# zellerlab/GECCO

Hardware: AMD Instinct MI355X
Metric: genes/sec CRF decode (windowed fwd-bwd marginals + Viterbi) (higher is better)
Workload: dtype f64

## Files before the change

gecco_amd/_native.py:

```python
import ctypes
import operator
import os
from typing import Optional, Sequence

import numpy as np

_HERE = os.path.dirname(os.path.abspath(__file__))
LIB_PATH = os.path.join(_HERE, "lib", "libgecco_crf.so")

OK, EINVAL, EFORMAT, ENOMEM, EHIP, ENODEV, EUNSUPPORTED = 0, -1, -2, -3, -4, -5, -6

_c_i32p = ctypes.POINTER(ctypes.c_int32)
_c_f64p = ctypes.POINTER(ctypes.c_double)
_c_u8p = ctypes.POINTER(ctypes.c_uint8)
_c_i8p = ctypes.POINTER(ctypes.c_int8)
_c_u32p = ctypes.POINTER(ctypes.c_uint32)
_vp = ctypes.c_void_p

SIGNATURES = {
    "gecco_crf_last_error": (ctypes.c_char_p, []),
    "gecco_crf_version": (ctypes.c_int, []),
    "gecco_crf_model_load": (ctypes.c_int, [ctypes.c_char_p, ctypes.c_size_t, ctypes.POINTER(_vp)]),
    "gecco_crf_model_from_tables": (ctypes.c_int, [_c_f64p, _c_f64p, ctypes.c_int32, ctypes.c_int32, ctypes.POINTER(_vp)]),
    "gecco_crf_model_free": (None, [_vp]),
# ... 103 lines not shown
         _c_f64p, _c_f64p, _c_f64p, _c_f64p, _c_f64p, _c_f64p],
    ),
    "gecco_crf_segment": (
        ctypes.c_int,
        [ctypes.c_int32, _c_f64p, _c_u8p, _c_i32p, ctypes.c_int32, ctypes.c_double, ctypes.c_int32, ctypes.c_int32,
         ctypes.c_int32, ctypes.c_int32, _c_i32p, ctypes.c_int32, _c_i32p],
    ),
    "gecco_crf_segment_ex": (
        ctypes.c_int, [ctypes.c_int32, _c_f64p, _c_u8p, _c_i32p, ctypes.c_int32, _vp, _c_i32p, ctypes.c_int32, _c_i32p]
    ),
    "gecco_crf_domain_composition": (
        ctypes.c_int,
        [ctypes.c_int32, _c_i32p, ctypes.c_int32, _c_i32p, ctypes.c_int32, _c_i32p, _c_f64p, ctypes.c_int32, ctypes.c_int32, _c_f64p],
    ),
    "gecco_crf_plan_create": (
        ctypes.c_int, [_vp, ctypes.c_int32, _c_i32p, ctypes.c_int32, ctypes.c_int32, ctypes.c_int32, ctypes.c_int32, ctypes.POINTER(_vp)]
    ),
    "gecco_crf_plan_free": (None, [_vp]),
    "gecco_crf_plan_num_genes": (ctypes.c_int32, [_vp]),
    "gecco_crf_plan_num_windows": (ctypes.c_int64, [_vp]),
    "gecco_crf_plan_num_tiles": (ctypes.c_int32, [_vp]),
    "gecco_crf_plan_tile_out": (ctypes.c_int32, [_vp]),
    "gecco_crf_plan_kernel_name": (ctypes.c_char_p, [_vp]),
    "gecco_crf_plan_run_windowed": (ctypes.c_int, [_vp, _vp, _vp, ctypes.c_int32, _vp, _vp]),
    "gecco_crf_plan_run_windowed_all": (ctypes.c_int, [_vp, _vp, _vp, ctypes.c_int32, _vp, _vp, _vp]),
    "gecco_crf_plan_all_kernel_name": (ctypes.c_char_p, [_vp]),
    "gecco_crf_plan_time_windowed_all": (
        ctypes.c_int, [_vp, _vp, _vp, ctypes.c_int32, _vp, _vp, _vp, ctypes.c_int32, ctypes.c_int32, ctypes.POINTER(ctypes.c_float)]
    ),
    "gecco_crf_plan_run_decode": (ctypes.c_int, [_vp, _vp, _vp, ctypes.c_int32, _vp, _vp, _vp, _vp]),
    "gecco_crf_plan_run_decode_pipelined": (ctypes.c_int, [_vp, _vp, _vp, ctypes.c_int32, _vp, _vp, _vp, _vp]),
    "gecco_crf_plan_run_marginals_full": (ctypes.c_int, [_vp, _vp, _vp, _vp, _vp, _vp]),
    "gecco_crf_plan_run_viterbi": (ctypes.c_int, [_vp, _vp, _vp, _vp, _vp, _vp]),
    "gecco_crf_plan_run_segment": (
        ctypes.c_int,
        [_vp, _vp, _vp, ctypes.c_double, ctypes.c_int32, ctypes.c_int32, ctypes.c_int32, ctypes.c_int32, _vp, ctypes.c_int32, _vp, _vp],
    ),
    "gecco_crf_plan_run_segment_ex": (ctypes.c_int, [_vp, _vp, _vp, _vp, _vp, ctypes.c_int32, _vp, _vp]),
    "gecco_crf_host_alloc": (ctypes.c_int, [ctypes.c_size_t, ctypes.POINTER(_vp)]),
    "gecco_crf_host_free": (None, [_vp]),
    "gecco_crf_session_create": (ctypes.c_int, [_vp, _c_i32p, ctypes.c_int32, ctypes.POINTER(_vp)]),
    "gecco_crf_session_free": (None, [_vp]),
    "gecco_crf_session_set_chunk_genes": (ctypes.c_int, [_vp, ctypes.c_int32]),
    "gecco_crf_session_set_direct_genes": (ctypes.c_int, [_vp, ctypes.c_int32]),
    "gecco_crf_session_stats": (
        ctypes.c_int,
# ... 1247 lines not shown
        if h:
            self._lib.gecco_crf_plan_free(h)

    @property
    def num_genes(self) -> int:
        return self._lib.gecco_crf_plan_num_genes(self._h)

    @property
    def num_windows(self) -> int:
        return self._lib.gecco_crf_plan_num_windows(self._h)

    @property
    def num_tiles(self) -> int:
        return self._lib.gecco_crf_plan_num_tiles(self._h)

    @property
    def tile_out(self) -> int:
        return self._lib.gecco_crf_plan_tile_out(self._h)

    @property
    def kernel_name(self) -> str:
        return self._lib.gecco_crf_plan_kernel_name(self._h).decode()

    def run_windowed(self, d_gene_ptr: int, d_attr_id: int, d_p_out: int, label=1, stream: int = 0):
        _check(self._lib.gecco_crf_plan_run_windowed(self._h, d_gene_ptr, d_attr_id, int(label), d_p_out, stream or None))

    @property
    def all_kernel_name(self) -> str:
        return self._lib.gecco_crf_plan_all_kernel_name(self._h).decode()

    def run_windowed_all(self, d_gene_ptr: int, d_attr_id: int, d_p_all: int, d_p_any: int = 0, background=None, stream: int = 0):
        _check(self._lib.gecco_crf_plan_run_windowed_all(self._h, d_gene_ptr, d_attr_id, -1 if background is None else int(background),
                                                         d_p_all, d_p_any or None, stream or None))

    def time_windowed_all(self, d_gene_ptr: int, d_attr_id: int, d_p_all: int, d_p_any: int = 0, background=None, stream: int = 0,
                          warmup=2, iters=10) -> float:
        ms = ctypes.c_float(0)
        _check(self._lib.gecco_crf_plan_time_windowed_all(self._h, d_gene_ptr, d_attr_id, -1 if background is None else int(background),
                                                          d_p_all, d_p_any or None, stream or None, int(warmup), int(iters),
                                                          ctypes.byref(ms)))
        return ms.value

    def run_decode(self, d_gene_ptr: int, d_attr_id: int, d_p_out: int, d_y: int, label: int = 1, d_score: int = 0, stream: int = 0):
        _check(self._lib.gecco_crf_plan_run_decode(self._h, d_gene_ptr, d_attr_id or None, int(label), d_p_out, d_y,
                                                   d_score or None, stream or None))

# ... 440 lines not shown
```

gecco_amd/csrc/capi.cpp:

```cpp
#include <cmath>
#include <cstdlib>
#include <cstring>
#include <exception>
#include <limits>
#include <memory>
#include <new>
#include <string>
#include <vector>

#include "../../include/gecco_crf.h"
#include "crf_exact_exp.hpp"
#include "crf_fisher.hpp"
#include "crf_forest.hpp"
#include "crf_model.hpp"
#include "crf_overlap.hpp"
#include "crf_plan.hpp"
#include "crf_session.hpp"
#include "crf_tables.hpp"
#include "crf_train.hpp"

using namespace gecco;

struct gecco_crf_model {
    Model m;
// ... 161 lines not shown
    }
    if (n_contigs > 0 && contig_ptr && contig_ptr[0] != 0) {
        set_error("contig_ptr[0] must be 0");
        return GECCO_CRF_EINVAL;
    }
    DeviceScope guard;
    GECCO_GUARD_BEGIN
    std::unique_ptr<gecco_crf_plan> h(new gecco_crf_plan());
    int rc = plan_build(m->m, device, contig_ptr, n_contigs, window, step, pad, h->p);
    if (rc) return rc;
    *out = h.release();
    return GECCO_CRF_OK;
    GECCO_GUARD_END
}
GECCO_API void gecco_crf_plan_free(gecco_crf_plan *p) {
    DeviceScope guard;
    delete p;
}
GECCO_API int32_t gecco_crf_plan_num_genes(const gecco_crf_plan *p) { return p ? p->p.n_genes : 0; }
GECCO_API int64_t gecco_crf_plan_num_windows(const gecco_crf_plan *p) { return p ? p->p.n_windows : 0; }
GECCO_API int32_t gecco_crf_plan_num_tiles(const gecco_crf_plan *p) { return p ? p->p.ntiles : 0; }
GECCO_API int32_t gecco_crf_plan_tile_out(const gecco_crf_plan *p) { return p ? p->p.tile_out : 0; }
GECCO_API const char *gecco_crf_plan_kernel_name(const gecco_crf_plan *p) { return p ? p->p.kernel_name.c_str() : ""; }

GECCO_API int gecco_crf_plan_run_windowed(gecco_crf_plan *p, const int32_t *d_gene_ptr, const int32_t *d_attr_id,
                                          int32_t label, double *d_p_out, void *stream) {
    if (!p) return GECCO_CRF_EINVAL;
    DeviceScope guard;
    GECCO_GUARD_BEGIN
    return plan_run_windowed(p->p, {d_gene_ptr, d_attr_id}, label, d_p_out, static_cast<hipStream_t>(stream));
    GECCO_GUARD_END
}

GECCO_API int gecco_crf_plan_run_windowed_all(gecco_crf_plan *p, const int32_t *d_gene_ptr, const int32_t *d_attr_id,
                                              int32_t background, double *d_p_all, double *d_p_any, void *stream) {
    if (!p) return GECCO_CRF_EINVAL;
    DeviceScope guard;
    GECCO_GUARD_BEGIN
    return plan_run_windowed_all(p->p, {d_gene_ptr, d_attr_id}, background, d_p_all, d_p_any, static_cast<hipStream_t>(stream));
    GECCO_GUARD_END
}
GECCO_API const char *gecco_crf_plan_all_kernel_name(const gecco_crf_plan *p) { return p ? plan_all_kernel_name(p->p) : ""; }

template <class Call>
static int time_calls(hipStream_t s, int32_t warmup, int32_t iters, float *ms_per_launch, Call call) {
    int rc;
// ... 2016 lines not shown
```

gecco_amd/csrc/crf_device.hpp:

```cpp
#pragma once
#include <hip/hip_runtime.h>

#include <cstddef>
#include <cstdint>

namespace gecco {

struct WinArgs {
    const int32_t *gene_ptr;
    const int32_t *attr_id;
    const double2 *wtab2;
    const double *wtab;
    const int32_t *c_slot;
    const int32_t *c_gene;
    const int32_t *c_n;
    const int4 *tile_desc;
    const uint64_t *start_bits;
    double *p_out;
    double2 *state_out;
    double *dstate_out;
    int32_t K, S, ntiles, W, step, L, label;
    int32_t n_genes, A;
    int32_t tiles_per_wg;
    int32_t all_regular;
    uint32_t rescale_mask;
    double mu01, rho, kappa_over_mu01, inv_kappa;
    double expc[12];
    double ratio_zmax;
    double g00, g01, g10, g11;
    int32_t generic;
    const double *exp_trans;
    double *scratch;
    const double *rtab;
    const double2 *ptab;
    int32_t prod_cnt;
    int32_t csr_end, csr_begin;
};

constexpr int kWinThreads = 256;
constexpr int kWinMaxW = 32;
constexpr int kWinTilesPerWg = 2;
constexpr int kWinTiles1MaxSlots = 350000;

__device__ __forceinline__ double exp_neg(double t, const double (&kExpC)[12]) {
    const double n = rint(t * 1.4426950408889634);
    double r = fma(n, 0.6931471805599453094, -t);
    r = fma(n, 2.3190468138462996e-17, r);
    double p = kExpC[0];
#pragma unroll
    for (int i = 1; i < 12; ++i) p = fma(p, r, kExpC[i]);
    p = fma(p, r, 1.0);
    p = fma(p, r, 1.0);
    return ldexp(p, -int(n));
}

__device__ __forceinline__ double exp_signed(double x, const double (&kExpC)[12]) {
    const double n = rint(x * 1.4426950408889634);
    double r = fma(-n, 0.6931471805599453094, x);
    r = fma(-n, 2.3190468138462996e-17, r);
// ... 311 lines not shown
```

gecco_amd/csrc/crf_kernels.hip:

```cpp
#include "crf_device.hpp"
#include "crf_lanes.hpp"
#include "crf_vd_short.hpp"

namespace gecco {
namespace {

typedef double f64x2 __attribute__((ext_vector_type(2)));

__device__ __forceinline__ double max_nocanon(double a, double b) {
    double r;
    asm("v_max_f64 %0, %1, %2" : "=v"(r) : "v"(a), "v"(b));
    return r;
}

__device__ __forceinline__ int xcd_remap(int orig, int nwg) {
    const int xcd = orig & 7, q = nwg >> 3, r = nwg & 7;
    const int base = xcd < r ? xcd * (q + 1) : r * (q + 1) + (xcd - r) * q;
    return base + (orig >> 3);
}

__device__ __forceinline__ void store_wt(double *p, double v) {
    __hip_atomic_store(reinterpret_cast<unsigned long long *>(p), static_cast<unsigned long long>(__double_as_longlong(v)),
                       __ATOMIC_RELAXED, __HIP_MEMORY_SCOPE_AGENT);
}

__device__ __forceinline__ double lds_read1(const double *p) {
    return __longlong_as_double(static_cast<long long>(
        __hip_atomic_load(reinterpret_cast<const unsigned long long *>(p), __ATOMIC_RELAXED, __HIP_MEMORY_SCOPE_WORKGROUP)));
}

__device__ __forceinline__ void rescale_pair(double &u, double &v) {
    int ex;
    (void)frexp(fmax(u, v), &ex);
    u = ldexp(u, -ex);
    v = ldexp(v, -ex);
}


constexpr int kGatherUnroll = 8;

template <int WMAX, int NT, int TT, bool EXACT>
struct WinSmem {
    static constexpr int JMAX = TT == 1 ? 2 : TT;
    static constexpr int CAP = TT == 1 ? NT + WMAX - 1 : TT * NT;
    static constexpr int CMAX = EXACT ? CAP / WMAX + 3 : CAP + 2;
    f64x2 ef[2 * CAP];
    uint32_t ginfo[CAP];
    f64x2 carry[NT / 64][WMAX];
    int32_t cslot[CMAX];
    int32_t cgene[CMAX];
    int32_t cn[CMAX];
};

struct SlotInfo {
    int gene;
    bool start_ok;
};

template <class Smem>
__device__ __forceinline__ SlotInfo slot_lookup(const Smem &sm, int cnt, int q, int S, int W, int step) {
    SlotInfo r{-1, false};
    if (q < 0 || q >= S) return r;
// ... 64 lines not shown
    using Smem = WinSmem<WMAX, NT, TT, EXACT>;
    constexpr int JMAX = Smem::JMAX;
    constexpr bool RATIO = !RESCALE && EXACT;
    const int W = EXACT ? WMAX : P.W;
    const int tid = threadIdx.x, lane = tid & 63, wave = tid >> 6;
    const int OUT = NT - (W - 1);
    const int ns = TT * OUT + 2 * (W - 1);
    const int q0 = tile * (TT * OUT) - (W - 1);

    const int4 td = P.all_regular ? make_int4(0, 0, 0, 1) : P.tile_desc[tile];
    int gene[JMAX];
    bool start[JMAX];
#pragma unroll
    for (int j = 0; j < JMAX; ++j) {
        gene[j] = -1;
        start[j] = false;
    }
    if (td.w & 1) {
#pragma unroll
        for (int j = 0; j < JMAX; ++j) {
            const int sl = tid + j * NT, q = q0 + sl;
            if (sl < ns && q >= 0 && q < P.S) {
                gene[j] = q + td.x;
                start[j] = (reinterpret_cast<const uint32_t *>(P.start_bits)[q >> 5] >> (q & 31)) & 1u;
            }
        }
    } else {
        const int cnt = td.z - td.y + 1;
        for (int j = tid; j <= cnt; j += NT) {
            sm.cslot[j] = P.c_slot[td.y + j];
            if (j < cnt) {
                sm.cgene[j] = P.c_gene[td.y + j];
                sm.cn[j] = P.c_n[td.y + j];
            }
        }
        __syncthreads();
#pragma unroll
        for (int j = 0; j < JMAX; ++j) {
            const int sl = tid + j * NT;
            if (sl < ns) {
                const SlotInfo si = slot_lookup(sm, cnt, q0 + sl, P.S, W, P.step);
                gene[j] = si.gene;
                start[j] = si.start_ok;
            }
        }
    }

// ... 30 lines not shown
        constexpr int SBASE = (Smem::CAP + 1) / 2;
        constexpr int APL = (2 * Smem::CAP - SBASE) / NT;
        constexpr int SCAP = APL * NT;
        static_assert(APL >= 1, "parking area smaller than one round of the workgroup");
        f64x2 *park = sm.ef + SBASE;
#pragma unroll 1
        for (uint32_t base = 0; base < n_attr; base += SCAP) {
            int id[APL];
#pragma unroll
            for (int a = 0; a < APL; ++a) id[a] = __builtin_amdgcn_raw_buffer_load_b32(ra, int((base + a * NT + tid) << 2), 0, 0);
            i32x4 w[APL];
#pragma unroll
            for (int a = 0; a < APL; ++a) {
                const uint32_t wo = min(uint32_t(id[a]), imax) << 4;
                w[a] = __builtin_amdgcn_raw_buffer_load_b128(rw, int(wo), 0, 0);
            }
#pragma unroll
            for (int a = 0; a < APL; ++a)
                park[a * NT + tid] = f64x2{__hiloint2double(w[a].y, w[a].x), __hiloint2double(w[a].w, w[a].z)};
            __syncthreads();
            const uint32_t c0 = lo_tile + base, c1 = c0 + SCAP;
#pragma unroll
            for (int j = 0; j < JMAX; ++j) {
                const f64x2 *k = park + (max(lo[j], c0) - c0);
                const f64x2 *const e = park + (min(hi[j], c1) - c0);
                for (; k < e && hi[j] > c0; ++k) {
                    const f64x2 v = *k;
                    if (RATIO) {
                        sc1[j] += v.x;
                        sc0[j] *= v.y;
                    } else {
                        sc0[j] += v.x;
                        sc1[j] += v.y;
                    }
                }
            }
            if (base + SCAP < n_attr) __syncthreads();
        }
        if (RATIO) {
#pragma unroll
            for (int j = 0; j < JMAX; ++j) long_run |= hi[j] - lo[j] > uint32_t(P.prod_cnt) ? 1u << j : 0u;
        }
        if (!RATIO && n_attr > 0) __syncthreads();
    } else {
        uint32_t off[JMAX], cnt[JMAX];
#pragma unroll
        for (int j = 0; j < JMAX; ++j) {
            int lo = 0, hi = 0;
            if (gene[j] >= 0) {
                lo = P.gene_ptr[gene[j]];
                hi = P.gene_ptr[gene[j] + 1];
            }
            off[j] = uint32_t(lo) - lo_tile;
            cnt[j] = uint32_t(hi - lo);
        }
        int ids[JMAX][kGatherUnroll];
#pragma unroll
// ... 31 lines not shown
            }
        }
    }
    if (RATIO) {
        if (__builtin_amdgcn_ballot_w64(long_run != 0) != 0) {
#pragma unroll
            for (int j = 0; j < JMAX; ++j)
                if ((long_run >> j) & 1u) sc0[j] = mu_exp_tab(sc1[j], P.rtab, P.expc);
        }
    }
    double *rr = reinterpret_cast<double *>(sm.ef);
#pragma unroll
    for (int j = 0; j < JMAX; ++j) {
        if (TT > 1 || j == 0 || wave == 0) {
            const int sl = tid + j * NT;
            const double s0 = sc0[j], s1 = sc1[j];
            if (sl >= W - 1 && sl < TT * OUT + (W - 1) && gene[j] >= 0) {
                if (!RATIO && P.state_out) reinterpret_cast<f64x2 *>(P.state_out)[gene[j]] = P.label ? f64x2{s0, s1} : f64x2{s1, s0};
            }
            const double d = RATIO ? s1 : s1 - s0;
            if (sl < ns) {
                if (RATIO) {
                    const double r = s0;
                    rr[sl] = __hiloint2double(__double2hiint(r) | (start[j] ? int(0x80000000u) : 0), __double2loint(r));
                    if (!(td.w & 1)) sm.ginfo[sl] = uint32_t(gene[j] + 1);
                } else {
                    const double e = exp_neg(fabs(d), P.expc);
                    const double e1 = d > 0.0 ? 1.0 : e;
                    sm.ef[sl] = f64x2{d > 0.0 ? e : 1.0, P.mu01 * e1};
                    sm.ginfo[sl] = (start[j] ? 0x80000000u : 0u) | uint32_t(gene[j] + 1);
                }
            }
        }
    }
    if (P.dstate_out) {
#pragma unroll
        for (int j = 0; j < JMAX; ++j) {
            if (TT > 1 || j == 0 || wave == 0) {
                const int sl = tid + j * NT;
                if (sl >= W - 1 && sl < TT * OUT + (W - 1) && gene[j] >= 0) {
                    const double d = RATIO ? sc1[j] : sc1[j] - sc0[j];
                    const double dd = __hiloint2double(__double2hiint(d) ^ (P.label ? 0 : int(0x80000000u)), __double2loint(d));
                    store_wt(P.dstate_out + gene[j], dd);
                }
            }
        }
    }
    __syncthreads();

    const uint32_t rmask = P.rescale_mask;
    const double rho = P.rho;
#pragma unroll 1
    for (int ph = 0; ph < TT; ++ph) {
        if (SMALL && ph > 0 && q0 + (W - 1) + ph * OUT >= P.S) break;
        const int sbase = ph * OUT + tid;
        bool my_start = false;
        int my_gene;
        if (RATIO) {
            const int q = q0 + sbase;
            my_gene = (td.w & 1) ? ((q >= 0 && q < P.S) ? q + td.x : -1) : int(sm.ginfo[sbase]) - 1;
        } else {
            const uint32_t gi = sm.ginfo[sbase];
            my_start = gi >> 31;
            my_gene = int(gi & 0x7fffffffu) - 1;
        }
        const f64x2 *ef = sm.ef + sbase;
        if constexpr (RATIO) {
            const double *rrs = rr + sbase;
            double A1[WMAX];
            const double r0 = lds_read1(rrs);
            double a0 = 1.0, a1 = fabs(r0) * P.kappa_over_mu01;
            A1[0] = a1;
#pragma unroll
            for (int k = 1; k < WMAX; ++k) {
                if (EXACT || k < W) {
                    const double r = fabs(lds_read1(rrs + k));
                    const double t = a0 + a1;
                    a1 = fma(a1, rho, a0) * r;
                    a0 = t;
                    A1[k] = a1;
                }
            }
            asm volatile("" ::: "memory");
            double z = fma(a1, P.inv_kappa, a0);
            const bool renorm = __builtin_amdgcn_ballot_w64(!(z < P.ratio_zmax)) != 0;
            auto pair_of = [&](double r, double &e0, double &f) {
                const bool pos = r > P.mu01;
                const double rc = fmin(r, 1.0e300);
                double q = __builtin_amdgcn_rcp(rc);
                q = fma(fma(-rc, q, 1.0), q, q);
// ... 2 lines not shown
            };
            if (renorm) {
                double e0, f;
                pair_of(fabs(r0), e0, f);
                a0 = e0;
                a1 = f * P.kappa_over_mu01;
                A1[0] = a1;
#pragma unroll
                for (int k = 1; k < WMAX; ++k) {
                    if (EXACT || k < W) {
                        pair_of(fabs(rrs[k]), e0, f);
                        const double t = a0 + a1;
                        a1 = fma(a1, rho, a0) * f;
                        a0 = t * e0;
                        A1[k] = a1;
                    }
                }
                z = fma(a1, P.inv_kappa, a0);
            }
            double b0, b1;
            {
                double r = __builtin_amdgcn_rcp(z);
                r = fma(fma(-z, r, 1.0), r, r);
                b0 = __double2hiint(r0) < 0 ? r : 0.0;
                b1 = b0 * P.inv_kappa;
            }
            double R = 0.0;
            double *carry = reinterpret_cast<double *>(&sm.carry[0][0]);
            if (!renorm) {
                double rcur = W > 1 ? lds_read1(rrs + (W - 1)) : 0.0;
#pragma unroll
                for (int k = WMAX - 1; k >= 0; --k) {
                    if (EXACT || k < W) {
                        double rnext = 0.0;
                        if (k > 1) rnext = lds_read1(rrs + (k - 1));
                        const double cand = A1[k] * b1;
                        if (k < W - 1) {
                            if (lane == 63 && wave < NT / 64 - 1) carry[wave * WMAX + k] = R;
                            R = wave_shr1_zero(R);
                        }
                        R = max_nocanon(R, cand);
                        if (k > 0) {
                            const double u = fabs(rcur) * b1;
                            b1 = fma(u, rho, b0);
                            b0 = b0 + u;
                        }
                        rcur = rnext;
                    }
                }
            } else {
#pragma unroll
                for (int k = WMAX - 1; k >= 0; --k) {
                    if (EXACT || k < W) {
                        const double cand = A1[k] * b1;
                        if (k < W - 1) {
                            if (lane == 63 && wave < NT / 64 - 1) carry[wave * WMAX + k] = R;
                            R = wave_shr1_zero(R);
                        }
                        R = max_nocanon(R, cand);
                        if (k > 0) {
                            double e0, f;
                            pair_of(fabs(rrs[k]), e0, f);
                            const double cc = e0 * b0, u = f * b1;
                            b0 = cc + u;
                            b1 = fma(u, rho, cc);
                        }
                    }
                }
            }
            __syncthreads();
            if (wave > 0 && lane < W - 1) {
                int t2 = tid;
                if (LEAN) asm volatile("" : "+v"(t2));
                R = fmax(R, carry[((t2 >> 6) - 1) * WMAX + (t2 & 63)]);
            }
            R = fmin(R, 1.0);
            if (tid >= W - 1 && my_gene >= 0) store_wt(P.p_out + my_gene, R);
        } else if constexpr (!RESCALE) {
            double A1[WMAX];
            double a0, a1;
            {
                const f64x2 c = ef[0];
                a0 = c.x;
                a1 = fabs(c.y) * P.kappa_over_mu01;
            }
            A1[0] = a1;
#pragma unroll
            for (int k = 1; k < WMAX; ++k) {
                if (EXACT || k < W) {
                    const f64x2 c = ef[k];
                    const double t = a0 + a1;
                    a1 = fma(a1, rho, a0) * fabs(c.y);
                    a0 = t * c.x;
                    A1[k] = a1;
                }
            }
            asm volatile("" ::: "memory");

            double b0, b1;
            {
// ... 84 lines not shown
            }
            if (tid >= W - 1 && my_gene >= 0) P.p_out[my_gene] = (Rx + Ry > 0.0) ? Rx / (Rx + Ry) : 0.0;
        }
        if (TT > 1) __syncthreads();
    }
}

template <int WMAX, bool EXACT, bool RESCALE, int NT, int TT>
__global__ void __launch_bounds__(NT, (RESCALE ? (WMAX <= 20 ? 5 : 3) : (WMAX <= 20 ? (TT <= 2 ? 8 : 5) : 3))) crf_windowed_l2(const WinArgs P) {
    __shared__ WinSmem<WMAX, NT, TT, EXACT> sm;
    windowed_tile<WMAX, EXACT, RESCALE, NT, TT>(P, sm, xcd_remap(blockIdx.x, P.ntiles));
}

__global__ void __launch_bounds__(kWinThreads, 4) crf_windowed_small_l2(const WinArgs P) {
    __shared__ WinSmem<20, kWinThreads, 2, true> sm;
    windowed_tile<20, true, false, kWinThreads, 2, false, true>(P, sm, 0);
}

struct PipeArgs {
    const int32_t *gene_ptr, *attr_id;
    const double2 *ptab;
    const int32_t *c_slot, *c_gene, *c_n;
    const int4 *tile_desc;
    const uint64_t *start_bits;
    double *p_out, *dstate_out;
    const double *rtab;
    int32_t S, ntiles, step, label, n_genes, A, all_regular, nvd8, prod_cnt;
    double mu01, rho, kappa_over_mu01, inv_kappa, ratio_zmax, expc5[5];
    const double *dstate;
    const uint8_t *flags;
    const uint16_t *lane_bits;
    const int32_t *cblk, *csr_gene_ptr, *csr_attr_id;
    const double2 *csr_wtab01;
    double2 *alpha;
    uint32_t *vd_stats;
    int8_t *y;
    int32_t s_n_genes, csr_n_attrs, v_exact, n_cblocks;
    double t00, t01, t10, t11, v_lo, v_hi, v_k, v_wmax2, v_tmax;
};

template <int TILES, int WGS>
__global__ void __launch_bounds__(kWinThreads, WGS) crf_decode_pipelined(const PipeArgs K) {
    using Smem = WinSmem<20, kWinThreads, TILES, true>;
    constexpr size_t kBytes = sizeof(Smem) > sizeof(VdShortSmem) ? sizeof(Smem) : sizeof(VdShortSmem);
    static_assert(kBytes <= 20480, "eight workgroups per CU");
    __shared__ __attribute__((aligned(16))) unsigned char raw[kBytes];
    const int b = blockIdx.x;
    if (b >= K.nvd8) {
        WinArgs P{};
        P.gene_ptr = K.gene_ptr;
        P.attr_id = K.attr_id;
        P.ptab = K.ptab;
        P.prod_cnt = K.prod_cnt;
        P.c_slot = K.c_slot;
        P.c_gene = K.c_gene;
        P.c_n = K.c_n;
        P.tile_desc = K.tile_desc;
        P.start_bits = K.start_bits;
        P.p_out = K.p_out;
        P.dstate_out = K.dstate_out;
        P.rtab = K.rtab;
        P.S = K.S;
        P.ntiles = K.ntiles;
        P.W = 20;
        P.step = K.step;
        P.L = 2;
        P.label = K.label;
        P.n_genes = K.n_genes;
        P.A = K.A;
        P.tiles_per_wg = TILES;
        P.all_regular = K.all_regular;
        P.mu01 = K.mu01;
        P.rho = K.rho;
        P.kappa_over_mu01 = K.kappa_over_mu01;
        P.inv_kappa = K.inv_kappa;
        P.ratio_zmax = K.ratio_zmax;
#pragma unroll
        for (int i = 0; i < 5; ++i) P.expc[7 + i] = K.expc5[i];
        P.csr_begin = P.csr_end = -1;
        windowed_tile<20, true, false, kWinThreads, TILES, true>(P, *reinterpret_cast<Smem *>(raw), xcd_remap(b - K.nvd8, K.ntiles));
        return;
// ... 143 lines not shown
    case 2: return launch_windowed_tt<2>(a, stream);
    case 3: return launch_windowed_tt<3>(a, stream);
    default: return hipErrorNotSupported;
    }
}

bool decode_pipelined_ok(const WinArgs &w, const SeqArgs &s) {
    return w.ntiles > 0 && w.W == 20 && w.rescale_mask == 0 && (w.tiles_per_wg == 1 || w.tiles_per_wg == 2) && !w.generic && w.L == 2 && !w.state_out && w.ptab &&
           s.short_contigs && s.n_cblocks > 0 && s.n_genes > 0;
}

hipError_t launch_decode_pipelined(const WinArgs &w, const SeqArgs &s, hipStream_t stream) {
    if (!decode_pipelined_ok(w, s)) return hipErrorNotSupported;
    PipeArgs k{};
    k.gene_ptr = w.gene_ptr;
    k.attr_id = w.attr_id;
    k.ptab = w.ptab;
    k.prod_cnt = w.prod_cnt;
    k.c_slot = w.c_slot;
    k.c_gene = w.c_gene;
    k.c_n = w.c_n;
    k.tile_desc = w.tile_desc;
    k.start_bits = w.start_bits;
    k.p_out = w.p_out;
    k.dstate_out = w.dstate_out;
    k.rtab = w.rtab;
    k.S = w.S;
    k.ntiles = w.ntiles;
    k.step = w.step;
    k.label = w.label;
    k.n_genes = w.n_genes;
    k.A = w.A;
    k.all_regular = w.all_regular;
    k.nvd8 = (s.n_cblocks + 7) & ~7;
    k.mu01 = w.mu01;
    k.rho = w.rho;
    k.kappa_over_mu01 = w.kappa_over_mu01;
    k.inv_kappa = w.inv_kappa;
    k.ratio_zmax = w.ratio_zmax;
    for (int i = 0; i < 5; ++i) k.expc5[i] = w.expc[7 + i];
    k.dstate = s.dstate;
    k.flags = s.flags;
    k.lane_bits = s.lane_bits;
    k.cblk = s.cblk;
    k.csr_gene_ptr = s.csr_gene_ptr;
    k.csr_attr_id = s.csr_attr_id;
// ... 32 lines not shown
```

gecco_amd/csrc/crf_plan.cpp:

```cpp
#include "crf_plan.hpp"

#include <algorithm>
#include <functional>
#include <memory>
#include <cmath>
#include <cstdio>
#include <cstdlib>
#include <cstring>

#include "../../include/gecco_crf.h"
#include "crf_session.hpp"

namespace gecco {

int check_hip(hipError_t e, const char *what) {
    if (e == hipSuccess) return GECCO_CRF_OK;
    set_error(std::string(what) + ": " + hipGetErrorString(e));
    if (e == hipErrorNoDevice || e == hipErrorInvalidDevice) return GECCO_CRF_ENODEV;
    if (e == hipErrorOutOfMemory) return GECCO_CRF_ENOMEM;
    return GECCO_CRF_EHIP;
}

Model::~Model() {
    for (auto &e : sessions) session_destroy(e.second);
// ... 298 lines not shown
            set_bit_range(start_bits, s0, int64_t(s0) + np - W + 1);
        } else {
            for (int32_t pos = 0; pos + W <= np; pos += step) {
                const int64_t q = int64_t(s0) + pos;
                start_bits[size_t(q >> 6)] |= 1ull << (q & 63);
            }
        }
        const bool padded = np != p.c_n[k];
        const bool gap_after = k + 1 < p.K && p.c_gene[k + 1] != p.c_gene[k] + p.c_n[k];
        irr_prefix[k + 1] = irr_prefix[k] + ((padded || gap_after) ? 1 : 0);
    }
    p.all_regular = p.skipped.empty() && p.S == p.n_genes && irr_prefix[size_t(p.K)] == 0;
    if (p.general && m.L >= 3 && gen_small_ok(m.L, W, m.trans.data()) && !std::getenv("GECCO_CRF_GENERAL_GROUPS")) {
        p.kernel_name = m.L > 8 ? "gl_windowed_mfma" : "gl_windowed_small";
        p.gen_small = true;
        p.tile_out = gen_small_tile_out(W);
    } else {
        p.kernel_name = p.reference_now ? "crf_windowed_reference_l2" : p.general ? "gl_windowed" : windowed_kernel_name(W, m.L, p.fast_ok);
        p.tile_out = windowed_tile_out(W, m.L, p.tiles_per_wg);
    }
    p.ntiles = p.S > 0 ? (p.S + p.tile_out - 1) / p.tile_out : 0;
    p.tile_desc.resize(p.ntiles);
    fill_tile_desc(p, irr_prefix, p.tile_out, p.ntiles, p.tile_desc.data());
    if (device < 0) return GECCO_CRF_OK;

    int rc = set_device(device);
    if (rc) return rc;
    if ((rc = get_device_tables(m, device, &p.tables_model))) return rc;
    Carver blk;
    auto take = [&](size_t bytes) { return blk.take(bytes ? bytes : 1); };
    const size_t o_slot = take(p.c_slot.size() * 4), o_gene = take(p.c_gene.size() * 4), o_n = take(p.c_n.size() * 4),
                 o_tile = take(p.tile_desc.size() * sizeof(int4)), o_bits = take(p.start_bits.size() * 8),
                 o_skip = take(p.skipped.size() * sizeof(int2)), o_cptr = take(p.contig_ptr.size() * 4);
    const size_t off = blk.off;
    if ((rc = p.tables.reserve(off, "plan tables"))) return rc;
    char *h = p.tables.h, *d = p.tables.d;
    if (p.tables_in_host_memory) {
        void *dv = nullptr;
        if ((rc = check_hip(hipHostGetDevicePointer(&dv, h, 0), "hipHostGetDevicePointer"))) return rc;
        d = static_cast<char *>(dv);
    }
    auto put = [&](size_t o, const void *src, size_t bytes) {
        if (bytes) std::memcpy(h + o, src, bytes);
    };
    put(o_slot, p.c_slot.data(), p.c_slot.size() * 4);
    put(o_gene, p.c_gene.data(), p.c_gene.size() * 4);
    put(o_n, p.c_n.data(), p.c_n.size() * 4);
    put(o_tile, p.tile_desc.data(), p.tile_desc.size() * sizeof(int4));
    put(o_bits, p.start_bits.data(), p.start_bits.size() * 8);
    put(o_skip, p.skipped.data(), p.skipped.size() * sizeof(int2));
    put(o_cptr, p.contig_ptr.data(), p.contig_ptr.size() * 4);
    p.d_c_slot = reinterpret_cast<int32_t *>(d + o_slot);
    p.d_c_gene = reinterpret_cast<int32_t *>(d + o_gene);
    p.d_c_n = reinterpret_cast<int32_t *>(d + o_n);
    p.d_tile_desc = reinterpret_cast<int4 *>(d + o_tile);
    p.d_start_bits = reinterpret_cast<uint64_t *>(d + o_bits) + 1;
    p.d_skipped = reinterpret_cast<int2 *>(d + o_skip);
    p.d_contig_ptr = reinterpret_cast<int32_t *>(d + o_cptr);
    if (p.tables_in_host_memory) return GECCO_CRF_OK;
    if (p.tables_by_kernel && !sync) {
        void *dv = nullptr;
        if ((rc = check_hip(hipHostGetDevicePointer(&dv, h, 0), "hipHostGetDevicePointer"))) return rc;
        return check_hip(launch_copy_block(dv, d, off, upload_stream), "plan tables launch");
    }
    if ((rc = check_hip(hipMemcpyAsync(d, h, off, hipMemcpyHostToDevice, upload_stream), "upload plan tables"))) return rc;
    if (sync && (rc = check_hip(hipStreamSynchronize(upload_stream), "upload plan tables"))) return rc;
    return GECCO_CRF_OK;
}

namespace {
constexpr int32_t kGenLongContig = 2048;

int fill_gen_args(Plan &p, const DeviceCsr &csr, GenArgs &a, bool whole_contig = false,
                  hipStream_t stream = nullptr, int32_t chunk_min_len = -1) {
    const Model &m = *p.model;
    const size_t n = size_t(p.n_genes), L = size_t(m.L);
    bool chunked = whole_contig;
    if (whole_contig)
        if (const char *env = std::getenv("GECCO_CRF_GENERAL_CHUNKED")) chunked = env[0] == '1';
// ... 324 lines not shown
        if ((rc = check_hip(hipMemsetAsync(d_p, 0, size_t(p.n_genes) * size_t(cols) * 8, stream), "memset p"))) return rc;
        if (d_p_any && (rc = check_hip(hipMemsetAsync(d_p_any, 0, size_t(p.n_genes) * 8, stream), "memset p"))) return rc;
    }
    if (!p.skipped.empty() &&
        (rc = check_hip(launch_all_fill_nan(d_p, d_p_any, cols, p.d_skipped, int(p.skipped.size()), stream), "fill_nan launch")))
        return rc;
    if (small) return check_hip(launch_gen_windowed_small(a, p.model->trans.data(), d_tiles, ntiles, stream), "windowed launch");
    return check_hip(launch_gen_windowed(a, stream), "windowed launch");
}
}

struct PipelinedLaunch {
    const SeqArgs *seq;
    bool *took = nullptr;
};
static int run_windowed_impl(Plan &p, const DeviceCsr &csr, int32_t label, double *d_p_out,
                             double2 *d_state_out, double *d_dstate_out, hipStream_t stream, const PipelinedLaunch *piped = nullptr);

int plan_run_windowed(Plan &p, const DeviceCsr &csr, int32_t label, double *d_p_out,
                      hipStream_t stream) {
    return run_windowed_impl(p, csr, label, d_p_out, nullptr, nullptr, stream);
}

static int run_windowed_impl(Plan &p, const DeviceCsr &csr, int32_t label, double *d_p_out,
                             double2 *d_state_out, double *d_dstate_out, hipStream_t stream, const PipelinedLaunch *piped) {
    int rc = check_plan(p, csr, label);
    if (rc || ends_here(p.n_genes == 0, !csr.gene_ptr || !d_p_out, rc)) return rc;
    if ((rc = use_device(p.device))) return rc;
    const Model &m = *p.model;
    if (p.general) return run_windowed_general(p, csr, label, -1, d_p_out, nullptr, p.gen_small, p.d_tile_desc, p.ntiles, stream);
    WinArgs a{};
    a.gene_ptr = csr.gene_ptr;
    a.attr_id = csr.attr_id;
    a.wtab = p.tables_model->wtab.get();
    a.wtab2 = p.tables_model->wtab2[label].get();
    a.exp_trans = p.tables_model->exp_trans.get();
    a.rtab = p.tables_model->rtab[label].get();
    a.ptab = p.tables_model->ptab[label].get();
    a.c_slot = p.d_c_slot;
    a.c_gene = p.d_c_gene;
    a.c_n = p.d_c_n;
    a.tile_desc = p.d_tile_desc;
    a.start_bits = p.d_start_bits;
    a.p_out = d_p_out;
    a.state_out = d_state_out;
    a.dstate_out = d_dstate_out;
    a.K = p.K;
    a.S = p.S;
    a.ntiles = p.ntiles;
    a.W = p.W;
    a.step = p.step;
    a.L = m.L;
    a.label = label;
    a.n_genes = p.n_genes;
    a.A = m.A;
    a.tiles_per_wg = p.tiles_per_wg;
    a.all_regular = p.all_regular ? 1 : 0;
    a.rescale_mask = p.rescale_mask;
    {
        const DeviceTables::WinConsts &c = p.tables_model->win[label];
        a.mu01 = c.mu01;
        a.rho = c.rho;
        a.kappa_over_mu01 = c.kappa_over_mu01;
        a.inv_kappa = c.inv_kappa;
        a.g00 = c.g00;
        a.g01 = c.g01;
// ... 716 lines not shown
```

gecco_amd/csrc/crf_plan.hpp:

```cpp
#pragma once
#include <hip/hip_runtime.h>

#include <cstdint>
#include <mutex>
#include <string>
#include <vector>

#include "crf_device.hpp"
#include "crf_hip_own.hpp"
#include "crf_model.hpp"

namespace gecco {

inline size_t align256(size_t x) { return (x + 255) & ~size_t(255); }

struct Carver {
    size_t off = 0;
    size_t take(size_t bytes) {
        const size_t at = off;
        off += align256(bytes);
        return at;
    }
};

// ... 26 lines not shown
    size_t cap = 0;
    int reserve(size_t bytes, const char *what);
    void release();
};

struct DeviceCsr {
    const int32_t *gene_ptr = nullptr, *attr_id = nullptr;
    const double *attr_value = nullptr;
    double vmax_abs = 1.0;
    const uint32_t *allowed = nullptr;
};

struct Plan {
    DeviceScope home{DeviceScope::kLater};
    const Model *model = nullptr;
    int device = -1;
    int32_t W = 0, step = 1, pad = 1;
    int32_t n_contigs = 0, n_genes = 0, n_max = 0;
    int64_t n_windows = 0;
    int32_t K = 0, S = 0, ntiles = 0, tile_out = 0, tiles_per_wg = 1;
    std::vector<int32_t> c_slot, c_gene, c_n;
    std::vector<int4> tile_desc;
    std::vector<uint64_t> start_bits;
    std::vector<int2> skipped;
    std::vector<int32_t> contig_ptr;
    std::vector<int32_t> irr_prefix;
    uint32_t rescale_mask = 0;
    bool all_regular = false;
    bool fast_ok = false;
    bool force_generic = false;
    bool general = false;
    bool gen_small = false;
    std::string kernel_name;
    Arena tables;
    int32_t *d_c_slot = nullptr, *d_c_gene = nullptr, *d_c_n = nullptr, *d_contig_ptr = nullptr;
    int4 *d_tile_desc = nullptr;
    uint64_t *d_start_bits = nullptr;
    int2 *d_skipped = nullptr;
    const DeviceTables *tables_model = nullptr;
    Arena seq;
    bool seq_ready = false;
    uint8_t *d_seq_flags = nullptr;
    const uint16_t *d_seq_flat_bits = nullptr;
    const uint16_t *d_seq_lane_bits = nullptr;
    int32_t *d_seq_cblk = nullptr;
    int32_t n_cblocks = 0;
    int32_t *d_seq_cblk_rank = nullptr, *d_seq_ne_contig = nullptr;
    int32_t n_empty_contigs = 0;
    bool seq_short = false;
    Stream side_stream;
    DeviceBlock<char> seq_ws, gen_ws, seg_ws;
    size_t vbound_sig = 0;
    DeviceBlock<double> win_scratch;
    struct GenTab {
        DeviceBlock<char> d;
        int32_t chunk = 0, min_len = -1;
        size_t nch = 0, off1 = 0, off2 = 0;
    } gen_tab[2];
    int32_t gen_wave_tmax = INT32_MIN, gen_wave_tmax_f = INT32_MIN;
    hipEvent_t ev_fork = nullptr, ev_join = nullptr;
// ... 7 lines not shown
    bool tables_in_host_memory = false;
    int64_t csr_begin = -1, csr_end = -1;
    bool reference_bits = false;
    bool windowed_use = true;
    bool reference_now = false;
    bool valued = false;
    bool masked = false;
    bool lattice = false;
    bool seq_in_host_memory = false;
    DeviceBlock<int4> all_tiles;
    int32_t all_ntiles = -1;
    std::mutex ws_mutex;
    ~Plan();
};

int plan_build(const Model &m, int device, const int32_t *contig_ptr, int32_t n_contigs, int32_t W, int32_t step,
               int32_t pad, Plan &p, hipStream_t upload_stream = nullptr, bool sync = true);
int plan_ensure_seq(Plan &p, hipStream_t stream, bool sync = true);
int plan_run_segment(Plan &p, const double *d_p, const uint8_t *d_annotated, const SegParams &params, int32_t *d_seg,
                     int32_t max_seg, int32_t *d_seg_off, int32_t *d_total, hipStream_t stream, double *d_gather = nullptr,
                     int32_t gather_cap = 0);
int plan_run_windowed(Plan &p, const DeviceCsr &csr, int32_t label, double *d_p_out,
                      hipStream_t stream);
int plan_run_windowed_all(Plan &p, const DeviceCsr &csr, int32_t background, double *d_p_all,
                          double *d_p_any, hipStream_t stream);
const char *plan_all_kernel_name(const Plan &p);
int plan_run_decode_pipelined(Plan *cur, const DeviceCsr &csr, int32_t label, double *d_p_out,
                              Plan *prev, int8_t *d_prev_y, hipStream_t stream);
int plan_run_decode(Plan &p, const DeviceCsr &csr, int32_t label, double *d_p_out,
                    int8_t *d_y, double *d_score, hipStream_t stream);
int plan_run_marginals_full(Plan &p, const DeviceCsr &csr, double *d_marg,
                            double *d_lognorm, hipStream_t stream);
int plan_run_viterbi(Plan &p, const DeviceCsr &csr, int8_t *d_y, double *d_score,
                     hipStream_t stream);
int plan_run_span_probabilities(Plan &p, const DeviceCsr &csr, const SpanQuery *d_spans, int32_t n_spans, double *d_logp,
                                double *d_marg, double *d_lognorm, hipStream_t stream);
int plan_run_span_conditionals(Plan &p, const DeviceCsr &csr, const ConditionalArgs &q, double *d_logp, double *d_marg,
                               double *d_lognorm, hipStream_t stream);
int plan_run_run_posteriors(Plan &p, const DeviceCsr &csr, const RunPosteriorArgs &q, double *d_marg, double *d_lognorm,
                            hipStream_t stream);
int plan_run_sample_paths(Plan &p, const DeviceCsr &csr, int32_t n_samples, uint64_t seed, const RunQuery *d_queries, int32_t n_runs,
                          int8_t *d_y, int32_t *d_runs, double *d_marg, double *d_lognorm, hipStream_t stream);
int plan_run_viterbi_kbest(Plan &p, const DeviceCsr &csr, int32_t k, uint16_t *d_back, uint16_t *d_fin, int8_t *d_y, double *d_score,
                           int32_t *d_n_paths, double *d_marg, double *d_lognorm, hipStream_t stream);
int plan_run_viterbi_min_run(Plan &p, const DeviceCsr &csr, uint32_t set_mask, int32_t min_run, uint8_t *d_back, int8_t *d_y,
                             double *d_score, double *d_lognorm_min_run, double *d_marg, double *d_lognorm, hipStream_t stream);
// ... 11 lines not shown
```

include/gecco_crf.h:

```cpp
#ifndef GECCO_CRF_H
#define GECCO_CRF_H

#include <stddef.h>
#include <stdint.h>

#ifdef __cplusplus
extern "C" {
#endif

#define GECCO_CRF_OK 0
#define GECCO_CRF_EINVAL (-1)
#define GECCO_CRF_EFORMAT (-2)
#define GECCO_CRF_ENOMEM (-3)
#define GECCO_CRF_EHIP (-4)
#define GECCO_CRF_ENODEV (-5)
#define GECCO_CRF_EUNSUPPORTED (-6)

typedef struct gecco_crf_model gecco_crf_model;
typedef struct gecco_crf_plan gecco_crf_plan;

const char *gecco_crf_last_error(void);
int gecco_crf_version(void);

int gecco_crf_model_load(const uint8_t *lcrf, size_t n_bytes, gecco_crf_model **out);
// ... 48 lines not shown
    int32_t trim;
    int32_t carry_state;
    const int32_t *marker_ptr;
    const int32_t *marker_id;
} gecco_crf_refine_params;
int gecco_crf_segment_ex(int32_t device, const double *p, const uint8_t *annotated,
                         const int32_t *contig_ptr, int32_t n_contigs, const gecco_crf_refine_params *params,
                         int32_t *seg_out, int32_t max_seg, int32_t *n_seg);

int gecco_crf_domain_composition(int32_t device, const int32_t *seg, int32_t n_seg,
                                 const int32_t *dom_ptr, int32_t n_genes,
                                 const int32_t *dom_col, const double *dom_weight,
                                 int32_t n_cols, int32_t normalize, double *comp_out);

int gecco_crf_plan_create(const gecco_crf_model *m, int32_t device,
                          const int32_t *contig_ptr , int32_t n_contigs,
                          int32_t window, int32_t step, int32_t pad, gecco_crf_plan **out);
void gecco_crf_plan_free(gecco_crf_plan *p);
int32_t gecco_crf_plan_num_genes(const gecco_crf_plan *p);
int64_t gecco_crf_plan_num_windows(const gecco_crf_plan *p);
int32_t gecco_crf_plan_num_tiles(const gecco_crf_plan *p);
int32_t gecco_crf_plan_tile_out(const gecco_crf_plan *p);
const char *gecco_crf_plan_kernel_name(const gecco_crf_plan *p);
int gecco_crf_plan_run_windowed(gecco_crf_plan *p, const int32_t *d_gene_ptr, const int32_t *d_attr_id,
                                int32_t label, double *d_p_out, void *stream);
int gecco_crf_plan_run_windowed_all(gecco_crf_plan *p, const int32_t *d_gene_ptr, const int32_t *d_attr_id,
                                    int32_t background, double *d_p_all, double *d_p_any, void *stream);
const char *gecco_crf_plan_all_kernel_name(const gecco_crf_plan *p);
int gecco_crf_plan_run_marginals_full(gecco_crf_plan *p, const int32_t *d_gene_ptr, const int32_t *d_attr_id,
                                      double *d_marg, double *d_lognorm, void *stream);
int gecco_crf_plan_run_viterbi(gecco_crf_plan *p, const int32_t *d_gene_ptr, const int32_t *d_attr_id,
                               int8_t *d_y, double *d_score, void *stream);
int gecco_crf_plan_run_decode(gecco_crf_plan *p, const int32_t *d_gene_ptr, const int32_t *d_attr_id,
                              int32_t label, double *d_p_out, int8_t *d_y, double *d_score, void *stream);
int gecco_crf_plan_run_decode_pipelined(gecco_crf_plan *p, const int32_t *d_gene_ptr, const int32_t *d_attr_id,
                                        int32_t label, double *d_p_out, gecco_crf_plan *prev, int8_t *d_prev_y,
                                        void *stream);
int gecco_crf_plan_run_segment(gecco_crf_plan *p, const double *d_p, const uint8_t *d_annotated,
                               double threshold, int32_t n_cds, int32_t edge_distance, int32_t trim,
                               int32_t carry_state, int32_t *d_seg, int32_t max_seg, int32_t *d_n_seg,
                               void *stream);
int gecco_crf_plan_run_segment_ex(gecco_crf_plan *p, const double *d_p, const uint8_t *d_annotated,
                                  const gecco_crf_refine_params *params, int32_t *d_seg, int32_t max_seg,
                                  int32_t *d_n_seg, void *stream);
int gecco_crf_plan_time_windowed(gecco_crf_plan *p, const int32_t *d_gene_ptr, const int32_t *d_attr_id,
                                 int32_t label, double *d_p_out, void *stream,
// ... 366 lines not shown
```

Measured before the change: 79.53 billion.

## Precompute per-wave phase start masks and block the parked-pair gather loop

Builds per-tile, per-phase, per-wave 64-bit start masks at plan time and uploads them. The ratio-form windowed kernel reads them through scalar constant loads and turns them into per-lane flags with inverse ballot, so it no longer packs a start bit into the sign of the LDS ratio value or loads start bits per slot. The parked-pair accumulation loop now loads four pairs at a time behind an opaque barrier, with a static check that over-reads stay inside LDS. Gene index computation is deferred to the store, and the last wave step skips a redundant shift and max. This adds plan-time host work and device memory for the masks, plus a debug readback API.

```diff
diff --git a/gecco_amd/_native.py b/gecco_amd/_native.py
--- a/gecco_amd/_native.py
+++ b/gecco_amd/_native.py
@@ -149,6 +149,7 @@
     "gecco_crf_plan_num_tiles": (ctypes.c_int32, [_vp]),
     "gecco_crf_plan_tile_out": (ctypes.c_int32, [_vp]),
     "gecco_crf_plan_kernel_name": (ctypes.c_char_p, [_vp]),
+    "gecco_crf_plan_phase_start_masks": (ctypes.c_int, [_vp, _vp, ctypes.c_int64, ctypes.POINTER(ctypes.c_int64)]),
     "gecco_crf_plan_run_windowed": (ctypes.c_int, [_vp, _vp, _vp, ctypes.c_int32, _vp, _vp]),
     "gecco_crf_plan_run_windowed_all": (ctypes.c_int, [_vp, _vp, _vp, ctypes.c_int32, _vp, _vp, _vp]),
     "gecco_crf_plan_all_kernel_name": (ctypes.c_char_p, [_vp]),
@@ -1442,6 +1443,14 @@
     def kernel_name(self) -> str:
         return self._lib.gecco_crf_plan_kernel_name(self._h).decode()
 
+    def phase_start_masks(self) -> np.ndarray:
+        n = ctypes.c_int64(0)
+        _check(self._lib.gecco_crf_plan_phase_start_masks(self._h, None, 0, ctypes.byref(n)))
+        out = np.zeros(n.value, dtype=np.uint64)
+        if n.value:
+            _check(self._lib.gecco_crf_plan_phase_start_masks(self._h, out.ctypes.data, n.value, ctypes.byref(n)))
+        return out.reshape(self.num_tiles, -1, 4) if n.value else out.reshape(0, 0, 4)
+
     def run_windowed(self, d_gene_ptr: int, d_attr_id: int, d_p_out: int, label=1, stream: int = 0):
         _check(self._lib.gecco_crf_plan_run_windowed(self._h, d_gene_ptr, d_attr_id, int(label), d_p_out, stream or None))
 
diff --git a/gecco_amd/csrc/capi.cpp b/gecco_amd/csrc/capi.cpp
--- a/gecco_amd/csrc/capi.cpp
+++ b/gecco_amd/csrc/capi.cpp
@@ -207,6 +207,13 @@
 GECCO_API int32_t gecco_crf_plan_num_tiles(const gecco_crf_plan *p) { return p ? p->p.ntiles : 0; }
 GECCO_API int32_t gecco_crf_plan_tile_out(const gecco_crf_plan *p) { return p ? p->p.tile_out : 0; }
 GECCO_API const char *gecco_crf_plan_kernel_name(const gecco_crf_plan *p) { return p ? p->p.kernel_name.c_str() : ""; }
+GECCO_API int gecco_crf_plan_phase_start_masks(gecco_crf_plan *p, uint64_t *out, int64_t cap, int64_t *n) {
+    if (!p || !n) return GECCO_CRF_EINVAL;
+    DeviceScope guard;
+    GECCO_GUARD_BEGIN
+    return plan_read_phase_start(p->p, out, cap, n);
+    GECCO_GUARD_END
+}
 
 GECCO_API int gecco_crf_plan_run_windowed(gecco_crf_plan *p, const int32_t *d_gene_ptr, const int32_t *d_attr_id,
                                           int32_t label, double *d_p_out, void *stream) {
diff --git a/gecco_amd/csrc/crf_device.hpp b/gecco_amd/csrc/crf_device.hpp
--- a/gecco_amd/csrc/crf_device.hpp
+++ b/gecco_amd/csrc/crf_device.hpp
@@ -35,6 +35,7 @@
     const double2 *ptab;
     int32_t prod_cnt;
     int32_t csr_end, csr_begin;
+    const uint64_t *phase_start;
 };
 
 constexpr int kWinThreads = 256;
diff --git a/gecco_amd/csrc/crf_kernels.hip b/gecco_amd/csrc/crf_kernels.hip
--- a/gecco_amd/csrc/crf_kernels.hip
+++ b/gecco_amd/csrc/crf_kernels.hip
@@ -38,6 +38,23 @@
 
 
 constexpr int kGatherUnroll = 8;
+constexpr int kRunBlock = 4;
+
+template <int U, class Acc>
+__device__ __forceinline__ void run_chain(const f64x2 (&v)[kRunBlock], int len, int t, Acc &acc) {
+    if constexpr (U < kRunBlock) {
+        if (len > t + U) {
+            asm volatile("");
+            acc(v[U]);
+            run_chain<U + 1>(v, len, t, acc);
+        }
+    }
+}
+
+__device__ __forceinline__ void run_block_opaque(f64x2 (&v)[kRunBlock]) {
+    static_assert(kRunBlock == 4, "one operand per pair of the block");
+    asm volatile("" : "+v"(v[0]), "+v"(v[1]), "+v"(v[2]), "+v"(v[3]));
+}
 
 template <int WMAX, int NT, int TT, bool EXACT>
 struct WinSmem {
@@ -148,7 +165,7 @@
             const int sl = tid + j * NT, q = q0 + sl;
             if (sl < ns && q >= 0 && q < P.S) {
                 gene[j] = q + td.x;
-                start[j] = (reinterpret_cast<const uint32_t *>(P.start_bits)[q >> 5] >> (q & 31)) & 1u;
+                if (!RATIO) start[j] = (reinterpret_cast<const uint32_t *>(P.start_bits)[q >> 5] >> (q & 31)) & 1u;
             }
         }
     } else {
@@ -225,10 +242,10 @@
             const uint32_t c0 = lo_tile + base, c1 = c0 + SCAP;
 #pragma unroll
             for (int j = 0; j < JMAX; ++j) {
-                const f64x2 *k = park + (max(lo[j], c0) - c0);
-                const f64x2 *const e = park + (min(hi[j], c1) - c0);
-                for (; k < e && hi[j] > c0; ++k) {
-                    const f64x2 v = *k;
+                const uint32_t b = max(lo[j], c0);
+                int rem = int(min(hi[j], c1) - b);
+                const f64x2 *k = park + (b - c0);
+                auto acc = [&](const f64x2 v) {
                     if (RATIO) {
                         sc1[j] += v.x;
                         sc0[j] *= v.y;
@@ -236,6 +253,16 @@
                         sc0[j] += v.x;
                         sc1[j] += v.y;
                     }
+                };
+                static_assert((SBASE + SCAP + kRunBlock - 1) * sizeof(f64x2) <= sizeof(Smem::ef) + sizeof(Smem::ginfo),
+                              "a block read past the last parked pair leaves the workgroup's LDS");
+                for (int t = 0; rem > t; t += kRunBlock, k += kRunBlock) {
+                    f64x2 v[kRunBlock];
+#pragma unroll
+                    for (int u = 0; u < kRunBlock; ++u) v[u] = k[u];
+                    run_block_opaque(v);
+                    acc(v[0]);
+                    run_chain<1>(v, rem, t, acc);
                 }
             }
             if (base + SCAP < n_attr) __syncthreads();
@@ -313,8 +340,12 @@
             if (sl < ns) {
                 if (RATIO) {
                     const double r = s0;
-                    rr[sl] = __hiloint2double(__double2hiint(r) | (start[j] ? int(0x80000000u) : 0), __double2loint(r));
-                    if (!(td.w & 1)) sm.ginfo[sl] = uint32_t(gene[j] + 1);
+                    if (td.w & 1) {
+                        rr[sl] = r;
+                    } else {
+                        rr[sl] = __hiloint2double(__double2hiint(r) | (start[j] ? int(0x80000000u) : 0), __double2loint(r));
+                        sm.ginfo[sl] = uint32_t(gene[j] + 1);
+                    }
                 } else {
                     const double e = exp_neg(fabs(d), P.expc);
                     const double e1 = d > 0.0 ? 1.0 : e;
@@ -348,8 +379,7 @@
         bool my_start = false;
         int my_gene;
         if (RATIO) {
-            const int q = q0 + sbase;
-            my_gene = (td.w & 1) ? ((q >= 0 && q < P.S) ? q + td.x : -1) : int(sm.ginfo[sbase]) - 1;
+            my_gene = -1;
         } else {
             const uint32_t gi = sm.ginfo[sbase];
             my_start = gi >> 31;
@@ -357,6 +387,13 @@
         }
         const f64x2 *ef = sm.ef + sbase;
         if constexpr (RATIO) {
+            uint64_t smask = 0;
+            if (td.w & 1) {
+                int wv = __builtin_amdgcn_readfirstlane(wave);
+                asm volatile("" : "+s"(wv));
+                typedef const __attribute__((address_space(4))) uint64_t *ConstMasks;
+                smask = reinterpret_cast<ConstMasks>(reinterpret_cast<uintptr_t>(P.phase_start))[(size_t(tile) * TT + size_t(ph)) * (NT / 64) + size_t(wv)];
+            }
             const double *rrs = rr + sbase;
             double A1[WMAX];
             const double r0 = lds_read1(rrs);
@@ -405,7 +442,11 @@
             {
                 double r = __builtin_amdgcn_rcp(z);
                 r = fma(fma(-z, r, 1.0), r, r);
-                b0 = __double2hiint(r0) < 0 ? r : 0.0;
+                if (td.w & 1) {
+                    b0 = __builtin_amdgcn_inverse_ballot_w64(smask) ? r : 0.0;
+                } else {
+                    b0 = __double2hiint(r0) < 0 ? r : 0.0;
+                }
                 b1 = b0 * P.inv_kappa;
             }
             double R = 0.0;
@@ -421,8 +462,10 @@
                         if (k < W - 1) {
                             if (lane == 63 && wave < NT / 64 - 1) carry[wave * WMAX + k] = R;
                             R = wave_shr1_zero(R);
+                            R = max_nocanon(R, cand);
+                        } else {
+                            R = cand;
                         }
-                        R = max_nocanon(R, cand);
                         if (k > 0) {
                             const double u = fabs(rcur) * b1;
                             b1 = fma(u, rho, b0);
@@ -458,7 +501,13 @@
                 R = fmax(R, carry[((t2 >> 6) - 1) * WMAX + (t2 & 63)]);
             }
             R = fmin(R, 1.0);
-            if (tid >= W - 1 && my_gene >= 0) store_wt(P.p_out + my_gene, R);
+            if (tid >= W - 1) {
+                int t3 = tid;
+                asm volatile("" : "+v"(t3));
+                const int sl = ph * OUT + t3, q = q0 + sl;
+                my_gene = (td.w & 1) ? ((q >= 0 && q < P.S) ? q + td.x : -1) : int(sm.ginfo[sl]) - 1;
+                if (my_gene >= 0) store_wt(P.p_out + my_gene, R);
+            }
         } else if constexpr (!RESCALE) {
             double A1[WMAX];
             double a0, a1;
@@ -589,7 +638,7 @@
     const double2 *ptab;
     const int32_t *c_slot, *c_gene, *c_n;
     const int4 *tile_desc;
-    const uint64_t *start_bits;
+    const uint64_t *start_bits, *phase_start;
     double *p_out, *dstate_out;
     const double *rtab;
     int32_t S, ntiles, step, label, n_genes, A, all_regular, nvd8, prod_cnt;
@@ -624,6 +673,7 @@
         P.c_n = K.c_n;
         P.tile_desc = K.tile_desc;
         P.start_bits = K.start_bits;
+        P.phase_start = K.phase_start;
         P.p_out = K.p_out;
         P.dstate_out = K.dstate_out;
         P.rtab = K.rtab;
@@ -813,6 +863,7 @@
     k.c_n = w.c_n;
     k.tile_desc = w.tile_desc;
     k.start_bits = w.start_bits;
+    k.phase_start = w.phase_start;
     k.p_out = w.p_out;
     k.dstate_out = w.dstate_out;
     k.rtab = w.rtab;
diff --git a/gecco_amd/csrc/crf_plan.cpp b/gecco_amd/csrc/crf_plan.cpp
--- a/gecco_amd/csrc/crf_plan.cpp
+++ b/gecco_amd/csrc/crf_plan.cpp
@@ -344,6 +344,22 @@
     p.ntiles = p.S > 0 ? (p.S + p.tile_out - 1) / p.tile_out : 0;
     p.tile_desc.resize(p.ntiles);
     fill_tile_desc(p, irr_prefix, p.tile_out, p.ntiles, p.tile_desc.data());
+    p.phase_start.clear();
+    if (p.fast_ok && windowed_ratio_form(W, p.rescale_mask)) {
+        constexpr int kWaves = kWinThreads / 64;
+        const int32_t tt = p.tiles_per_wg, out = kWinThreads - (W - 1);
+        p.phase_start.resize(size_t(p.ntiles) * size_t(tt) * kWaves);
+        const uint64_t *const words = p.start_bits.data();
+        size_t i = 0;
+        for (int32_t b = 0; b < p.ntiles; ++b)
+            for (int32_t ph = 0; ph < tt; ++ph)
+                for (int w = 0; w < kWaves; ++w, ++i) {
+                    const int64_t bit = int64_t(b) * p.tile_out - (W - 1) + int64_t(ph) * out + 64 * w + 64;
+                    const size_t k = size_t(bit >> 6);
+                    const int s = int(bit & 63);
+                    p.phase_start[i] = s ? (words[k] >> s) | (words[k + 1] << (64 - s)) : words[k];
+                }
+    }
     if (device < 0) return GECCO_CRF_OK;
 
     int rc = set_device(device);
@@ -353,6 +369,7 @@
     auto take = [&](size_t bytes) { return blk.take(bytes ? bytes : 1); };
     const size_t o_slot = take(p.c_slot.size() * 4), o_gene = take(p.c_gene.size() * 4), o_n = take(p.c_n.size() * 4),
                  o_tile = take(p.tile_desc.size() * sizeof(int4)), o_bits = take(p.start_bits.size() * 8),
+                 o_phase = take(p.phase_start.size() * 8),
                  o_skip = take(p.skipped.size() * sizeof(int2)), o_cptr = take(p.contig_ptr.size() * 4);
     const size_t off = blk.off;
     if ((rc = p.tables.reserve(off, "plan tables"))) return rc;
@@ -370,6 +387,7 @@
     put(o_n, p.c_n.data(), p.c_n.size() * 4);
     put(o_tile, p.tile_desc.data(), p.tile_desc.size() * sizeof(int4));
     put(o_bits, p.start_bits.data(), p.start_bits.size() * 8);
+    put(o_phase, p.phase_start.data(), p.phase_start.size() * 8);
     put(o_skip, p.skipped.data(), p.skipped.size() * sizeof(int2));
     put(o_cptr, p.contig_ptr.data(), p.contig_ptr.size() * 4);
     p.d_c_slot = reinterpret_cast<int32_t *>(d + o_slot);
@@ -377,6 +395,7 @@
     p.d_c_n = reinterpret_cast<int32_t *>(d + o_n);
     p.d_tile_desc = reinterpret_cast<int4 *>(d + o_tile);
     p.d_start_bits = reinterpret_cast<uint64_t *>(d + o_bits) + 1;
+    p.d_phase_start = p.phase_start.empty() ? nullptr : reinterpret_cast<uint64_t *>(d + o_phase);
     p.d_skipped = reinterpret_cast<int2 *>(d + o_skip);
     p.d_contig_ptr = reinterpret_cast<int32_t *>(d + o_cptr);
     if (p.tables_in_host_memory) return GECCO_CRF_OK;
@@ -747,6 +766,19 @@
     return run_windowed_impl(p, csr, label, d_p_out, nullptr, nullptr, stream);
 }
 
+int plan_read_phase_start(Plan &p, uint64_t *out, int64_t cap, int64_t *n) {
+    *n = int64_t(p.phase_start.size());
+    if (!out || p.phase_start.empty()) return GECCO_CRF_OK;
+    if (cap < *n || !p.d_phase_start) {
+        set_error(cap < *n ? "buffer too small for the plan's phase masks" : "the plan has no device tables");
+        return GECCO_CRF_EINVAL;
+    }
+    int rc = use_device(p.device);
+    if (rc) return rc;
+    if ((rc = check_hip(hipDeviceSynchronize(), "hipDeviceSynchronize"))) return rc;
+    return check_hip(hipMemcpy(out, p.d_phase_start, size_t(*n) * 8, hipMemcpyDefault), "read phase masks");
+}
+
 static int run_windowed_impl(Plan &p, const DeviceCsr &csr, int32_t label, double *d_p_out,
                              double2 *d_state_out, double *d_dstate_out, hipStream_t stream, const PipelinedLaunch *piped) {
     int rc = check_plan(p, csr, label);
@@ -767,6 +799,7 @@
     a.c_n = p.d_c_n;
     a.tile_desc = p.d_tile_desc;
     a.start_bits = p.d_start_bits;
+    a.phase_start = p.d_phase_start;
     a.p_out = d_p_out;
     a.state_out = d_state_out;
     a.dstate_out = d_dstate_out;
diff --git a/gecco_amd/csrc/crf_plan.hpp b/gecco_amd/csrc/crf_plan.hpp
--- a/gecco_amd/csrc/crf_plan.hpp
+++ b/gecco_amd/csrc/crf_plan.hpp
@@ -72,6 +72,7 @@
     std::vector<int32_t> c_slot, c_gene, c_n;
     std::vector<int4> tile_desc;
     std::vector<uint64_t> start_bits;
+    std::vector<uint64_t> phase_start;
     std::vector<int2> skipped;
     std::vector<int32_t> contig_ptr;
     std::vector<int32_t> irr_prefix;
@@ -85,7 +86,7 @@
     Arena tables;
     int32_t *d_c_slot = nullptr, *d_c_gene = nullptr, *d_c_n = nullptr, *d_contig_ptr = nullptr;
     int4 *d_tile_desc = nullptr;
-    uint64_t *d_start_bits = nullptr;
+    uint64_t *d_start_bits = nullptr, *d_phase_start = nullptr;
     int2 *d_skipped = nullptr;
     const DeviceTables *tables_model = nullptr;
     Arena seq;
@@ -139,6 +140,7 @@
                      int32_t gather_cap = 0);
 int plan_run_windowed(Plan &p, const DeviceCsr &csr, int32_t label, double *d_p_out,
                       hipStream_t stream);
+int plan_read_phase_start(Plan &p, uint64_t *out, int64_t cap, int64_t *n);
 int plan_run_windowed_all(Plan &p, const DeviceCsr &csr, int32_t background, double *d_p_all,
                           double *d_p_any, hipStream_t stream);
 const char *plan_all_kernel_name(const Plan &p);
diff --git a/include/gecco_crf.h b/include/gecco_crf.h
--- a/include/gecco_crf.h
+++ b/include/gecco_crf.h
@@ -94,6 +94,7 @@
 int32_t gecco_crf_plan_num_tiles(const gecco_crf_plan *p);
 int32_t gecco_crf_plan_tile_out(const gecco_crf_plan *p);
 const char *gecco_crf_plan_kernel_name(const gecco_crf_plan *p);
+int gecco_crf_plan_phase_start_masks(gecco_crf_plan *p, uint64_t *out, int64_t cap, int64_t *n);
 int gecco_crf_plan_run_windowed(gecco_crf_plan *p, const int32_t *d_gene_ptr, const int32_t *d_attr_id,
                                 int32_t label, double *d_p_out, void *stream);
 int gecco_crf_plan_run_windowed_all(gecco_crf_plan *p, const int32_t *d_gene_ptr, const int32_t *d_attr_id,
```

Result: no change. 78.85 billion (-0.9%).
